# gregc-91/GPU-Raytracing

Hardware: AMD Instinct MI355X
Metric: Mrays/s at 1920x1080 primary rays + BVH build ms, 1M-tri scene (higher is better)
Workload: dtype f32; 1 GPU; grid_mesh(G=708, seed=1) = 1002528 triangles, 1920x1080, 1 spp, camera A (top-down), render_type 0; LBVH replicated per GPU; parallelism=row-bands x1, 8 frames in flight on 8 HIP streams

## Files before the change

gpu-raytracing_amd/csrc/rt_traverse.hpp:

```cpp
#pragma once

#include "rt_device.hpp"
#include "rt_math.h"

namespace rt {

constexpr int kStackLds = 16;
constexpr int kStackMax = 64;
constexpr uint32_t kPrefetchMinPrims = 8u << 20;
#ifndef RT_TRACE_WAVES
#define RT_TRACE_WAVES 4
#endif
constexpr int kTraceWaves = RT_TRACE_WAVES;
#ifndef RT_TRACE_MIN_WAVES
#define RT_TRACE_MIN_WAVES 7
#endif
#ifndef RT_TRACE_LEAN_EXTRA
#define RT_TRACE_LEAN_EXTRA 1
#endif
#ifndef RT_TRACE_PF_WAVES
#define RT_TRACE_PF_WAVES 5
#endif

#ifndef RT_TRACE_UNIFORM_MAX
#define RT_TRACE_UNIFORM_MAX 0
#endif
constexpr int kUniformMax = RT_TRACE_UNIFORM_MAX;
#ifndef RT_TRACE_UNIFORM_STICKY
#define RT_TRACE_UNIFORM_STICKY 1
#endif
constexpr bool kUniformSticky = RT_TRACE_UNIFORM_STICKY != 0;
#ifndef RT_TRACE_PAIR_BARRIER
#define RT_TRACE_PAIR_BARRIER 0
#endif
#ifndef RT_TRACE_LEAF_WIDE
#define RT_TRACE_LEAF_WIDE 1
#endif

constexpr int kParkNum = 8, kParkDen = 1;

#ifndef RT_TRACE_XCD_CHUNK
#define RT_TRACE_XCD_CHUNK 8
#endif
__device__ __forceinline__ uint32_t xcd_chunk_block(uint32_t bid, uint32_t nb)
{
    constexpr uint32_t kXcdChunk = RT_TRACE_XCD_CHUNK;
    const uint32_t full = nb / (8u * kXcdChunk) * (8u * kXcdChunk);
    const uint32_t xcd = bid & 7u, loc = bid >> 3;
    return bid < full ? (loc / kXcdChunk) * (8u * kXcdChunk) + xcd * kXcdChunk + (loc % kXcdChunk) : bid;
}

typedef __attribute__((address_space(3))) uint32_t lds_u32;

struct Ray {
    float ox, oy, oz, dx, dy, dz, ix, iy, iz, tmin, tmax;
};
struct Hit {
    uint32_t primitive_id, tri_id;
    float bu, bv;
};

struct NoFilter {
    static constexpr bool active = false;
};

template <class Filter = NoFilter>
__device__ __forceinline__ bool intersect_tri(float v0x, float v0y, float v0z, float v1x, float v1y, float v1z,
                                              float v2x, float v2y, float v2z, Ray& r, Hit& h, uint32_t tri_id,
                                              uint32_t prim_id, Filter flt = Filter())
{
    const float epsilon = 0.000000001f;
    const float e1x = v1x - v0x, e1y = v1y - v0y, e1z = v1z - v0z;
    const float e2x = v2x - v0x, e2y = v2y - v0y, e2z = v2z - v0z;
    const float hx = r.dy * e2z - r.dz * e2y, hy = r.dz * e2x - r.dx * e2z, hz = r.dx * e2y - r.dy * e2x;
    const float a = e1x * hx + e1y * hy + e1z * hz;
    if (a > -epsilon && a < epsilon) return false;
    const float f = 1.0f / a;
    const float sx = r.ox - v0x, sy = r.oy - v0y, sz = r.oz - v0z;
    const float u = f * (sx * hx + sy * hy + sz * hz);
    if (u < 0.0f || u > 1.0f) return false;
    const float qx = sy * e1z - sz * e1y, qy = sz * e1x - sx * e1z, qz = sx * e1y - sy * e1x;
    const float v = f * (r.dx * qx + r.dy * qy + r.dz * qz);
    if (v < 0.0f || (u + v) > 1.0f) return false;
    const float t = f * (e2x * qx + e2y * qy + e2z * qz);
    if (t < r.tmin || t > r.tmax) return false;
    if constexpr (Filter::active) {
        if (!flt.keep(a, prim_id)) return false;
    }
    r.tmax = t;
    h.primitive_id = prim_id;
    h.tri_id = tri_id;
    h.bu = u;
    h.bv = v;
    return true;
}

#ifndef RT_TRACE_QUAD_WAIT
#define RT_TRACE_QUAD_WAIT 1
#endif

#ifndef RT_TRACE_QUAD_WAIT_SECOND
#define RT_TRACE_QUAD_WAIT_SECOND 0
#endif

#ifndef RT_TRACE_LEAN_STEP
#define RT_TRACE_LEAN_STEP 2
#endif
constexpr int kLeanStep = RT_TRACE_LEAN_STEP;
constexpr int kLeanMargin = 4;
#ifndef RT_TRACE_LEAN_SELECT
#define RT_TRACE_LEAN_SELECT 0
#endif
constexpr bool kLeanSelect = RT_TRACE_LEAN_SELECT != 0;
#ifndef RT_TRACE_HOLD_VECTOR
#define RT_TRACE_HOLD_VECTOR 0
#endif
static_assert(kLeanMargin <= kStackLds, "the lean vote's threshold is a stack level");

enum : uint32_t { PH_STEP = 0, PH_LEAF0 = 1, PH_LEAF1 = 2, PH_DONE = 3, PH_STEP_POP = 4 };
constexpr uint32_t kNoNear = 0xFFFFFFFFu;

typedef uint32_t SpillArray[kStackMax - kStackLds];

struct Trav {
    lds_u32* lds;
    uint32_t* spill;
    int sp;
    uint32_t cur;
    uint32_t near_e;
    float near_d;
    uint32_t phase;
    uint32_t leaf;
    float f1, k1;
    uint32_t e1;
    uint32_t t1;
    uint32_t box_tests, tri_tests;
    uint4 pf0, pf1, pf2, pf3;

    template <int LEAN = 0>
    __device__ __forceinline__ void push(uint32_t e, bool lean = false)
    {
        if constexpr (LEAN == 1) { lds[sp * 64] = e; sp++; return; }
        if (LEAN == 2 && lean) { lds[sp * 64] = e; sp++; return; }
        if (sp < kStackLds) lds[sp * 64] = e;
        else if (sp < kStackMax) spill[sp - kStackLds] = e;
        sp = min(sp + 1, kStackMax);
    }
    template <int LEAN = 0>
    __device__ __forceinline__ void inner_hit(bool in, uint32_t e, float front, bool lean = false)
    {
        const bool closer = (front < near_d) | ((front == near_d) & ((e & kIndexMask) > (near_e & kIndexMask)));
        if (in & (near_e != kNoNear)) push<LEAN>(closer ? near_e : e, lean);
        const bool take = in & closer;
        near_e = take ? e : near_e;
        near_d = take ? front : near_d;
    }
    template <bool QW = false, int LEAN = 0>
    __device__ __forceinline__ void advance(bool lean = false)
    {
        const uint32_t cnt = cur >> 29;
        if constexpr (LEAN == 1 && kLeanSelect) {
            const bool more = cnt > 2, keep = near_e != kNoNear;
            const bool pop = !more & !keep & (sp != 0);
            cur = more ? ((cur & kIndexMask) + 2) | ((cnt - 2) << 29) : (keep ? near_e : cur);
            phase = (more | keep | pop) ? phase : (uint32_t)PH_DONE;
            near_e = more ? near_e : kNoNear;
            near_d = more ? near_d : __builtin_inff();
            if (pop) { --sp; cur = lds[sp * 64]; if constexpr (QW) phase = PH_STEP_POP; }
            return;
        }
        if (cnt > 2) { cur = ((cur & kIndexMask) + 2) | ((cnt - 2) << 29); return; }
        const bool keep = LEAN == 1 ? near_e != kNoNear : (near_e != kNoNear) & (sp < kStackMax);
        if (keep) cur = near_e;
        else if (sp == 0) phase = PH_DONE;
        else {
            --sp;
            if (LEAN == 1 || (LEAN == 2 && lean)) cur = lds[sp * 64];
            else cur = sp < kStackLds ? lds[sp * 64] : spill[sp - kStackLds];
            if constexpr (QW) phase = PH_STEP_POP;
        }
        near_e = kNoNear;
        near_d = __builtin_inff();
    }
    template <int LEAN = 0>
    __device__ __forceinline__ void second_slot(float tmin, float tmax, bool lean = false)
    {
        const bool valid = t1 != RT_CHILD_NONE;
        const bool hit = valid & (k1 >= f1) & (f1 <= tmax) & (k1 >= tmin);
        box_tests += valid ? 1u : 0u;
        const bool is_leaf = hit & (t1 == RT_CHILD_TRI);
        inner_hit<LEAN>(hit & !is_leaf, e1, f1, lean);
        if (is_leaf) { leaf = e1; phase = PH_LEAF1; }
    }
};

__device__ __forceinline__ void slab(const uint4& a, const uint4& b, const Ray& r, float& front, float& back)
{
    typedef float v2f __attribute__((ext_vector_type(2)));
    const v2f o2 = {r.ox, r.oy}, i2 = {r.ix, r.iy};
    const v2f lo = {__uint_as_float(a.x), __uint_as_float(a.y)}, hi = {__uint_as_float(b.x), __uint_as_float(b.y)};
    const v2f t1 = (lo - o2) * i2, t2 = (hi - o2) * i2;
    const float t1z = (__uint_as_float(a.z) - r.oz) * r.iz, t2z = (__uint_as_float(b.z) - r.oz) * r.iz;
    front = fmaxf(fmaxf(fminf(t1.x, t2.x), fminf(t1.y, t2.y)), fminf(t1z, t2z));
    back = fminf(fminf(fmaxf(t1.x, t2.x), fmaxf(t1.y, t2.y)), fmaxf(t1z, t2z));
}

template <bool PF, class Params>
__device__ __forceinline__ void prefetch_pair(const Params& p, Trav& t)
{
    if constexpr (PF) {
        if (t.phase == PH_STEP) {
            const uint4* np = reinterpret_cast<const uint4*>(p.nodes + (t.cur & kIndexMask));
            const int o1 = (t.cur >> 29) > 1 ? 2 : 0;
            t.pf0 = np[0]; t.pf1 = np[1]; t.pf2 = np[o1]; t.pf3 = np[o1 + 1];
        }
    }
}

template <bool PF, bool QW = false, int LEAN = 0, class Params>
__device__ __forceinline__ void box_step_on(const Params& p, const Ray& r, Trav& t, bool two, const uint4& a0, const uint4& b0,
                                            const uint4& a1, const uint4& b1, bool lean = false)
{
    if constexpr (QW) t.phase = PH_STEP;
    float f0, k0;
    slab(a0, b0, r, f0, k0);
    slab(a1, b1, r, t.f1, t.k1);
    t.e1 = (b1.w & kIndexMask) | (a1.w & ~kIndexMask);
    t.t1 = two ? (b1.w >> 29) : (uint32_t)RT_CHILD_NONE;
    const uint32_t type0 = b0.w >> 29;
    const uint32_t e0 = (b0.w & kIndexMask) | (a0.w & ~kIndexMask);
    const bool valid0 = type0 != RT_CHILD_NONE;
    const bool hit0 = valid0 & (k0 >= f0) & (f0 <= r.tmax) & (k0 >= r.tmin);
    t.box_tests += valid0 ? 1u : 0u;
    const bool leaf0 = hit0 & (type0 == RT_CHILD_TRI);
    t.template inner_hit<LEAN>(hit0 & !leaf0, e0, f0, lean);
    if (leaf0) { t.leaf = e0; t.phase = PH_LEAF0; }
    else {
        t.template second_slot<LEAN>(r.tmin, r.tmax, lean);
        if (t.phase == PH_STEP) { t.template advance<QW, LEAN>(lean); prefetch_pair<PF>(p, t); }
    }
}

template <bool PF, bool QW = false, int LEAN = 0, class Params>
__device__ __forceinline__ void box_step(const Params& p, const Ray& r, Trav& t, bool lean = false)
{
    const uint32_t cnt = t.cur >> 29;
    const uint4* np = reinterpret_cast<const uint4*>(p.nodes + (t.cur & kIndexMask));
#ifdef RT_EXP_BOX_PAD
#pragma unroll
    for (int q = 0; q < RT_EXP_BOX_PAD; q++) asm volatile("v_mov_b32 %0, %0" : "+v"(t.box_tests));
#endif
    const bool two = cnt > 1;
    const int o1 = two ? 2 : 0;
    uint4 a0, b0, a1, b1;
    if constexpr (PF) { a0 = t.pf0; b0 = t.pf1; a1 = t.pf2; b1 = t.pf3; }
    else {
        a0 = np[0]; b0 = np[1]; a1 = np[o1]; b1 = np[o1 + 1];
#if RT_TRACE_PAIR_BARRIER
        __builtin_amdgcn_sched_barrier(0);
#endif
    }
    box_step_on<PF, QW, LEAN>(p, r, t, two, a0, b0, a1, b1, lean);
}

template <bool ANY>
__device__ __forceinline__ bool quad_hold(const Trav& t)
{
    const bool popped = t.phase == PH_STEP_POP && t.sp < kStackLds;
    const int key = ANY && t.phase == PH_DONE ? 0 : t.sp;
    const int k0 = __builtin_amdgcn_mov_dpp(key, 0x00, 0xF, 0xF, true), k1 = __builtin_amdgcn_mov_dpp(key, 0x55, 0xF, 0xF, true);
    const int k2 = __builtin_amdgcn_mov_dpp(key, 0xAA, 0xF, 0xF, true), k3 = __builtin_amdgcn_mov_dpp(key, 0xFF, 0xF, 0xF, true);
    bool hold = false;
    if (popped) {
        typedef uint32_t lds_u32x4 __attribute__((ext_vector_type(4)));
        typedef __attribute__((address_space(3))) lds_u32x4 lds_quad;
        const lds_u32x4 e = *(const lds_quad*)(((uintptr_t)t.lds & ~(uintptr_t)15) + (uintptr_t)t.sp * 256u);
#if RT_TRACE_HOLD_VECTOR
        hold = max(max(e.x == t.cur ? k0 : 0, e.y == t.cur ? k1 : 0), max(e.z == t.cur ? k2 : 0, e.w == t.cur ? k3 : 0)) > t.sp;
#else
        hold = ((k0 > t.sp) & (e.x == t.cur)) | ((k1 > t.sp) & (e.y == t.cur)) | ((k2 > t.sp) & (e.z == t.cur)) |
               ((k3 > t.sp) & (e.w == t.cur));
#endif
    }
    return hold;
}

template <bool PF, bool ANY, int LEAN, class Params>
__device__ __forceinline__ void quad_vote_steps(const Params& p, const Ray& r, Trav& t, bool go, bool lean)
{
    if (go) box_step<PF, true, LEAN>(p, r, t, lean);
#if RT_TRACE_QUAD_WAIT_SECOND
    if (((t.phase & 3u) == PH_STEP) & !quad_hold<ANY>(t)) box_step<PF, true, LEAN>(p, r, t, lean);
#else
    if ((t.phase & 3u) == PH_STEP) box_step<PF, true, LEAN>(p, r, t, lean);
#endif
}

typedef uint32_t u32x4 __attribute__((ext_vector_type(4)));
typedef const __attribute__((address_space(4))) u32x4* const_u4_ptr;
template <class Params>
__device__ __forceinline__ void box_step_shared(const Params& p, const Ray& r, Trav& t, uint32_t c)
{
    c = (uint32_t)__builtin_amdgcn_readfirstlane((int)c);
    const const_u4_ptr np = (const_u4_ptr)(uintptr_t)(p.nodes + (c & kIndexMask));
    const bool two = (c >> 29) > 1;
    const int o1 = two ? 2 : 0;
    const u32x4 a0 = np[0], b0 = np[1], a1 = np[o1], b1 = np[o1 + 1];
    box_step_on<false>(p, r, t, two, make_uint4(a0.x, a0.y, a0.z, a0.w), make_uint4(b0.x, b0.y, b0.z, b0.w),
                       make_uint4(a1.x, a1.y, a1.z, a1.w), make_uint4(b1.x, b1.y, b1.z, b1.w));
}

template <bool PF, class Params>
__device__ __forceinline__ bool box_step_wave(const Params& p, const Ray& r, Trav& t, uint64_t st)
{
    if constexpr (!PF && kUniformMax > 0) {
        constexpr int K = kUniformMax > 0 ? kUniformMax : 1;
        uint32_t cs[K];
        uint64_t ms[K];
        uint64_t rest = st;
#pragma unroll
        for (int k = 0; k < kUniformMax; k++) {
            cs[k] = 0; ms[k] = 0;
            if (rest) {
                cs[k] = (uint32_t)__builtin_amdgcn_readlane((int)t.cur, __ffsll((unsigned long long)rest) - 1);
                ms[k] = __builtin_amdgcn_ballot_w64(t.phase == PH_STEP && t.cur == cs[k]);
                rest &= ~ms[k];
            }
        }
        if (rest == 0) {
#pragma unroll
            for (int k = 0; k < kUniformMax; k++)
                if (ms[k]) { if (t.phase == PH_STEP && t.cur == cs[k]) box_step_shared(p, r, t, cs[k]); }
            return true;
        }
    }
    if (t.phase == PH_STEP) box_step<PF>(p, r, t);
    return false;
}

template <bool PF, bool ANY = false, bool QW = false, class Params, class Filter = NoFilter>
__device__ __forceinline__ bool trace_ray(const Params& p, Ray& r, Hit& h, Trav& t, bool active, uint32_t* steps,
                                          Filter flt = Filter())
{
    static_assert(!(PF && QW), "prefetch_pair tests phase == PH_STEP: a PH_STEP_POP lane would step on a stale prefetched pair");
    t.sp = 0;
    t.cur = (p.root & kIndexMask) | (p.count << 29);
    t.near_e = kNoNear;
    t.near_d = __builtin_inff();
    t.phase = (active && p.count > 0) ? PH_STEP : PH_DONE;
    t.box_tests = 0;
    t.tri_tests = 0;
    t.t1 = 0;
    t.e1 = 0;
    t.f1 = t.k1 = 0.0f;
    t.leaf = 0;
    prefetch_pair<PF>(p, t);
    bool tri_hit = false;
    uint32_t nbox = 0, nleaf = 0;
    bool lean = false;
    bool shared = true;
#ifdef RT_EXP_UNIFORM_STATS
    uint32_t ustat[4] = {0, 0, 0, 0};
#endif

    while (true) {
        uint64_t stepping, parked;
        while (true) {
            if constexpr (QW) {
                const bool go = ((t.phase & 3u) == PH_STEP) & !quad_hold<ANY>(t);
                stepping = __builtin_amdgcn_ballot_w64(go);
                parked = __builtin_amdgcn_ballot_w64((t.phase - 1u) < 2u);
                if constexpr (kLeanStep != 0)
                    lean = __builtin_amdgcn_ballot_w64((t.sp > kStackLds - kLeanMargin) & !(ANY && t.phase == PH_DONE)) == 0;
                if (stepping == 0 || __popcll(stepping) * p.park_den < __popcll(parked) * p.park_num) break;
                nbox += 2;
                if constexpr (kLeanStep == 1) {
                    if (lean) quad_vote_steps<PF, ANY, 1>(p, r, t, go, true);
                    else quad_vote_steps<PF, ANY, 0>(p, r, t, go, false);
                } else quad_vote_steps<PF, ANY, kLeanStep>(p, r, t, go, lean);
                continue;
            }
            stepping = __builtin_amdgcn_ballot_w64(t.phase == PH_STEP);
            parked = __builtin_amdgcn_ballot_w64((t.phase - 1u) < 2u);
            if (stepping == 0 || __popcll(stepping) * p.park_den < __popcll(parked) * p.park_num) break;
            nbox += 2;
#ifdef RT_EXP_UNIFORM_STATS
            {
                uint64_t rest = stepping;
                int distinct = 0;
                while (rest && distinct < 5) {
                    const int l0 = __ffsll((unsigned long long)rest) - 1;
                    const uint32_t c0 = (uint32_t)__builtin_amdgcn_readlane((int)t.cur, l0);
                    rest &= ~__builtin_amdgcn_ballot_w64(t.phase == PH_STEP && t.cur == c0);
                    distinct++;
                }
                ustat[distinct <= 1 ? 0 : (distinct == 2 ? 1 : (distinct <= 4 ? 2 : 3))]++;
            }
#endif
            if constexpr (!PF && kUniformMax > 0) {
                if (!kUniformSticky || shared) {
                    shared = box_step_wave<PF>(p, r, t, stepping);
                    const uint64_t again = __builtin_amdgcn_ballot_w64(t.phase == PH_STEP);
                    if (again) shared = box_step_wave<PF>(p, r, t, again);
                    continue;
                }
            }
            if (t.phase == PH_STEP) box_step<PF>(p, r, t);
            if (t.phase == PH_STEP) box_step<PF>(p, r, t);
        }
        if ((stepping | parked) == 0) break;
        nleaf++;
        if ((t.phase - 1u) < 2u) {
            t.tri_tests++;
            const uint32_t li = t.leaf & kIndexMask;
            const uint4* tp = reinterpret_cast<const uint4*>(p.leaves + li);
            uint4 l0 = tp[0], l1 = tp[1], l2 = tp[2], l3 = tp[3];
#if RT_TRACE_LEAF_WIDE
            asm volatile("" : "+v"(l0.x), "+v"(l0.y), "+v"(l0.z), "+v"(l0.w), "+v"(l1.x), "+v"(l1.y), "+v"(l1.z), "+v"(l1.w),
                              "+v"(l2.x), "+v"(l2.y), "+v"(l2.z), "+v"(l2.w), "+v"(l3.x), "+v"(l3.y), "+v"(l3.z), "+v"(l3.w));
#endif
            bool hit_tri = intersect_tri(__uint_as_float(l0.x), __uint_as_float(l0.y), __uint_as_float(l0.z),
                                         __uint_as_float(l1.x), __uint_as_float(l1.y), __uint_as_float(l1.z),
                                         __uint_as_float(l2.x), __uint_as_float(l2.y), __uint_as_float(l2.z),
                                         r, h, li << 1, l0.w, flt);
            if ((t.leaf >> 29) > 0 && (l3.x != l2.x || l3.y != l2.y || l3.z != l2.z))
                hit_tri |= intersect_tri(__uint_as_float(l2.x), __uint_as_float(l2.y), __uint_as_float(l2.z),
                                         __uint_as_float(l1.x), __uint_as_float(l1.y), __uint_as_float(l1.z),
                                         __uint_as_float(l3.x), __uint_as_float(l3.y), __uint_as_float(l3.z),
                                         r, h, (li << 1) + 1, l1.w, flt);
            tri_hit |= hit_tri;
            if (ANY && hit_tri) {
                t.phase = PH_DONE;
            } else {
                const bool was_first = t.phase == PH_LEAF0;
                t.phase = PH_STEP;
                if (QW && kLeanStep == 1 && lean) {
                    if (was_first) t.template second_slot<1>(r.tmin, r.tmax);
                    if (t.phase == PH_STEP) t.template advance<QW, 1>();
                } else if constexpr (QW && kLeanStep == 2) {
                    if (was_first) t.template second_slot<2>(r.tmin, r.tmax, lean);
                    if (t.phase == PH_STEP) t.template advance<QW, 2>(lean);
                } else {
                    if (was_first) t.second_slot(r.tmin, r.tmax);
                    if (t.phase == PH_STEP) { t.template advance<QW>(); prefetch_pair<PF>(p, t); }
                }
            }
        }
    }
#ifdef RT_EXP_UNIFORM_STATS
    steps[0] += ustat[RT_EXP_UNIFORM_STATS == 1 ? 0 : 2];
    steps[1] += ustat[RT_EXP_UNIFORM_STATS == 1 ? 1 : 3];
    (void)nbox; (void)nleaf;
#elif !defined(RT_TRACE_NO_STEPS)
    steps[0] += nbox;
    steps[1] += nleaf;
#endif
    return tri_hit;
}

__device__ __forceinline__ void camera_ray(const rt_camera& cam, uint32_t w, uint32_t h, uint32_t x, uint32_t y, float ox,
                                           float oy, Ray& r)
{
    const float ndcx = 2 * (((float)x + ox) / (float)w) - 1;
    const float ndcy = 2 * (((float)y + oy) / (float)h) - 1;
    const float px = (ndcx * cam.u.x + ndcy * cam.v.x) + 1.0f * cam.w.x;
    const float py = (ndcx * cam.u.y + ndcy * cam.v.y) + 1.0f * cam.w.y;
    const float pz = (ndcx * cam.u.z + ndcy * cam.v.z) + 1.0f * cam.w.z;
    const float inv_len = 1.0f / sqrtf(px * px + py * py + pz * pz);
    r.dx = px * inv_len; r.dy = py * inv_len; r.dz = pz * inv_len;
    r.ox = cam.position.x; r.oy = cam.position.y; r.oz = cam.position.z;
    r.tmin = 0.00001f;
    r.tmax = cam.max_depth;
}

__device__ __forceinline__ void subpixel_offset(uint32_t s, uint32_t spp, float& ox, float& oy)
{
    const uint32_t side = spp == 4 ? 2u : 4u;
    ox = ((float)(s % side) + 0.5f) / (float)side;
    oy = ((float)((s / side) % side) + 0.5f) / (float)side;
}

}
```

Measured before the change: 1191 Mrays/s.

## Add fused pair-step fast path for quad-vote traversal when no lane needs wide state

Adds a specialized box-step variant that tests both children of a node in one pass, pushing the farther hit and moving directly to the nearer one. It skips the deferred second-slot machinery. A wave-wide ballot picks this narrow path only when no active lane has more than two children pending or a saved near entry; otherwise the original step runs. This aims to cut per-step instruction count and phase bookkeeping in the common case, at the cost of an extra ballot per iteration and larger code size from the added template instantiations.

```diff
diff --git a/gpu-raytracing_amd/csrc/rt_traverse.hpp b/gpu-raytracing_amd/csrc/rt_traverse.hpp
--- a/gpu-raytracing_amd/csrc/rt_traverse.hpp
+++ b/gpu-raytracing_amd/csrc/rt_traverse.hpp
@@ -117,6 +117,11 @@
 #endif
 static_assert(kLeanMargin <= kStackLds, "the lean vote's threshold is a stack level");
 
+#ifndef RT_TRACE_PAIR_STEP
+#define RT_TRACE_PAIR_STEP 1
+#endif
+constexpr int kPairStep = RT_TRACE_PAIR_STEP;
+
 enum : uint32_t { PH_STEP = 0, PH_LEAF0 = 1, PH_LEAF1 = 2, PH_DONE = 3, PH_STEP_POP = 4 };
 constexpr uint32_t kNoNear = 0xFFFFFFFFu;
 
@@ -241,7 +246,57 @@
     }
 }
 
-template <bool PF, bool QW = false, int LEAN = 0, class Params>
+template <int LEAN, bool TAIL>
+__device__ __forceinline__ void pair_step_on(const Ray& r, Trav& t, bool two, const uint4& a0, const uint4& b0, const uint4& a1,
+                                             const uint4& b1, bool lean)
+{
+    t.phase = PH_STEP;
+    float f0, k0, f1, k1;
+    slab(a0, b0, r, f0, k0);
+    slab(a1, b1, r, f1, k1);
+    const uint32_t e0 = (b0.w & kIndexMask) | (a0.w & ~kIndexMask), e1 = (b1.w & kIndexMask) | (a1.w & ~kIndexMask);
+    const uint32_t type0 = b0.w >> 29, type1 = two ? (b1.w >> 29) : (uint32_t)RT_CHILD_NONE;
+    const bool valid0 = type0 != RT_CHILD_NONE, valid1 = type1 != RT_CHILD_NONE;
+    const bool hit0 = valid0 & (k0 >= f0) & (f0 <= r.tmax) & (k0 >= r.tmin);
+    t.box_tests += valid0 ? 1u : 0u;
+    t.f1 = f1; t.k1 = k1; t.e1 = e1; t.t1 = type1;
+    if (hit0 & (type0 == RT_CHILD_TRI)) {
+        t.leaf = e0; t.phase = PH_LEAF0;
+        return;
+    }
+    const bool hit1 = valid1 & (k1 >= f1) & (f1 <= r.tmax) & (k1 >= r.tmin);
+    t.box_tests += valid1 ? 1u : 0u;
+    const bool leaf1 = hit1 & (type1 == RT_CHILD_TRI), box1 = hit1 & !leaf1;
+    const bool closer = (f1 < f0) | ((f1 == f0) & ((e1 & kIndexMask) > (e0 & kIndexMask)));
+    if (hit0 & box1) t.template push<LEAN>(closer ? e0 : e1, lean);
+    const bool second = box1 & (closer | !hit0);
+    const uint32_t near = second ? e1 : (hit0 ? e0 : kNoNear);
+    const float nd = second ? f1 : (hit0 ? f0 : __builtin_inff());
+    if (leaf1) {
+        t.near_e = near; t.near_d = nd;
+        t.leaf = e1; t.phase = PH_LEAF1;
+        return;
+    }
+    if constexpr (TAIL) {
+        const uint32_t cnt = t.cur >> 29;
+        if (cnt > 2) {
+            t.near_e = near; t.near_d = nd;
+            t.cur = ((t.cur & kIndexMask) + 2) | ((cnt - 2) << 29);
+            return;
+        }
+    }
+    const bool keep = LEAN == 1 ? near != kNoNear : (near != kNoNear) & (t.sp < kStackMax);
+    if (keep) t.cur = near;
+    else if (t.sp == 0) t.phase = PH_DONE;
+    else {
+        --t.sp;
+        if (LEAN == 1 || (LEAN == 2 && lean)) t.cur = t.lds[t.sp * 64];
+        else t.cur = t.sp < kStackLds ? t.lds[t.sp * 64] : t.spill[t.sp - kStackLds];
+        t.phase = PH_STEP_POP;
+    }
+}
+
+template <bool PF, bool QW = false, int LEAN = 0, int PAIR = 0, class Params>
 __device__ __forceinline__ void box_step(const Params& p, const Ray& r, Trav& t, bool lean = false)
 {
     const uint32_t cnt = t.cur >> 29;
@@ -260,7 +315,8 @@
         __builtin_amdgcn_sched_barrier(0);
 #endif
     }
-    box_step_on<PF, QW, LEAN>(p, r, t, two, a0, b0, a1, b1, lean);
+    if constexpr (QW && PAIR != 0) pair_step_on<LEAN, PAIR == 2>(r, t, two, a0, b0, a1, b1, lean);
+    else box_step_on<PF, QW, LEAN>(p, r, t, two, a0, b0, a1, b1, lean);
 }
 
 template <bool ANY>
@@ -285,14 +341,14 @@
     return hold;
 }
 
-template <bool PF, bool ANY, int LEAN, class Params>
+template <bool PF, bool ANY, int LEAN, bool NARROW = false, class Params>
 __device__ __forceinline__ void quad_vote_steps(const Params& p, const Ray& r, Trav& t, bool go, bool lean)
 {
-    if (go) box_step<PF, true, LEAN>(p, r, t, lean);
+    if (go) box_step<PF, true, LEAN, NARROW ? 1 : 0>(p, r, t, lean);
 #if RT_TRACE_QUAD_WAIT_SECOND
-    if (((t.phase & 3u) == PH_STEP) & !quad_hold<ANY>(t)) box_step<PF, true, LEAN>(p, r, t, lean);
+    if (((t.phase & 3u) == PH_STEP) & !quad_hold<ANY>(t)) box_step<PF, true, LEAN, NARROW ? 2 : 0>(p, r, t, lean);
 #else
-    if ((t.phase & 3u) == PH_STEP) box_step<PF, true, LEAN>(p, r, t, lean);
+    if ((t.phase & 3u) == PH_STEP) box_step<PF, true, LEAN, NARROW ? 2 : 0>(p, r, t, lean);
 #endif
 }
 
@@ -374,10 +430,23 @@
                     lean = __builtin_amdgcn_ballot_w64((t.sp > kStackLds - kLeanMargin) & !(ANY && t.phase == PH_DONE)) == 0;
                 if (stepping == 0 || __popcll(stepping) * p.park_den < __popcll(parked) * p.park_num) break;
                 nbox += 2;
-                if constexpr (kLeanStep == 1) {
-                    if (lean) quad_vote_steps<PF, ANY, 1>(p, r, t, go, true);
-                    else quad_vote_steps<PF, ANY, 0>(p, r, t, go, false);
-                } else quad_vote_steps<PF, ANY, kLeanStep>(p, r, t, go, lean);
+                uint64_t wide = ~0ull;
+                if constexpr (kPairStep != 0) {
+                    wide = __builtin_amdgcn_ballot_w64((t.phase != PH_DONE) & (((t.cur >> 29) > 2) | (t.near_e != kNoNear)));
+                    if (wide == 0) {
+                        if constexpr (kLeanStep == 1) {
+                            if (lean) quad_vote_steps<PF, ANY, 1, true>(p, r, t, go, true);
+                            else quad_vote_steps<PF, ANY, 0, true>(p, r, t, go, false);
+                        } else quad_vote_steps<PF, ANY, kLeanStep, true>(p, r, t, go, lean);
+                    }
+                    asm volatile("" : "+s"(wide));
+                }
+                if (wide != 0) {
+                    if constexpr (kLeanStep == 1) {
+                        if (lean) quad_vote_steps<PF, ANY, 1>(p, r, t, go, true);
+                        else quad_vote_steps<PF, ANY, 0>(p, r, t, go, false);
+                    } else quad_vote_steps<PF, ANY, kLeanStep>(p, r, t, go, lean);
+                }
                 continue;
             }
             stepping = __builtin_amdgcn_ballot_w64(t.phase == PH_STEP);
```

After: 1232 Mrays/s, median of 6. 3.5% higher.
